# lightkurve/lightkurve

Hardware: AMD Instinct MI355X
Metric: frequencies*targets/sec (Lomb-Scargle, ls_method='fast' (reference default): extirpolation + FFT) + BLS periods*targets/sec; max-power rel-err (higher is better)
Workload: dtype f64

## Files before the change

### lightkurve_amd/csrc/ls_epilogue.hpp

```cpp
#pragma once
#include <hip/hip_runtime.h>

#include "../../include/lkhip.h"

namespace lk {

__device__ __forceinline__ double gls_power_sums(double Sh, double Ch, double S, double C, double S2, double C2,
                                                 int fit_mean, int norm, double YY, double psd_factor, double nN,
                                                 double scale) {
    double tan2;
    if (fit_mean)
        tan2 = (S2 - 2.0 * S * C) / (C2 - (C * C - S * S));
    else
        tan2 = S2 / C2;
    const double C2w = 1.0 / sqrt(1.0 + tan2 * tan2);
    const double S2w = tan2 * C2w;
    const double Cw = sqrt(0.5) * sqrt(1.0 + C2w);
    const double sgn = (S2w > 0.0) ? 1.0 : ((S2w < 0.0) ? -1.0 : 0.0);
    const double Sw = sqrt(0.5) * sgn * sqrt(1.0 - C2w);
    const double YC = Ch * Cw + Sh * Sw;
    const double YS = Sh * Cw - Ch * Sw;
    double CC = 0.5 * (1.0 + C2 * C2w + S2 * S2w);
    double SS = 0.5 * (1.0 - C2 * C2w - S2 * S2w);
    if (fit_mean) {
        const double a = C * Cw + S * Sw, bq = S * Cw - C * Sw;
        CC -= a * a;
        SS -= bq * bq;
    }
    double p = YC * YC / CC + YS * YS / SS;
    switch (norm) {
        case LK_NORM_STANDARD: p /= YY; break;
        case LK_NORM_PSD: p *= psd_factor; break;
        case LK_NORM_LK_AMPLITUDE: p = sqrt(p * psd_factor) * sqrt(4.0 / nN); break;
        default: p = p * psd_factor * scale; break;
    }
    return p;
}

__host__ __device__ __forceinline__ double rsqrt_refined(double x) {
#if defined(__HIP_DEVICE_COMPILE__)
    const double y = __builtin_amdgcn_rsq(x);
    const double e = fma(-(x * y), y, 1.0);
    return fma(y * e, fma(0.375, e, 0.5), y);
#else
    return 1.0 / sqrt(x);
#endif
}

__device__ __forceinline__ double gls_power_sums_lean(double Sh, double Ch, double S, double C, double S2, double C2,
                                                      int fit_mean, int norm, double YY, double psd_factor, double nN,
                                                      double scale) {
    double num = S2, den = C2;
    if (fit_mean) {
        num = S2 - 2.0 * S * C;
        den = C2 - (C * C - S * S);
    }
    double C2w, S2w;
    if (fmax(fabs(num), fabs(den)) >= 1e-150) {
        const double r = rsqrt_refined(num * num + den * den);
        C2w = fabs(den) * r;
        S2w = (den == 0.0) ? NAN : ((den < 0.0) ? -num : num) * r;
    } else {
        const double tan2 = num / den;
        C2w = 1.0 / sqrt(1.0 + tan2 * tan2);
        S2w = tan2 * C2w;
    }
    const double u = 0.5 + 0.5 * C2w;
    const double rc = rsqrt_refined(u);
    const double Cw = u * rc;
    const double Sw = 0.5 * S2w * rc;
    const double YC = Ch * Cw + Sh * Sw;
    const double YS = Sh * Cw - Ch * Sw;
    double CC = 0.5 * (1.0 + C2 * C2w + S2 * S2w);
    double SS = 0.5 * (1.0 - C2 * C2w - S2 * S2w);
    if (fit_mean) {
        const double a = C * Cw + S * Sw, bq = S * Cw - C * Sw;
        CC -= a * a;
        SS -= bq * bq;
    }
    double p = YC * YC / CC + YS * YS / SS;
    switch (norm) {
        case LK_NORM_STANDARD: p /= YY; break;
        case LK_NORM_PSD: p *= psd_factor; break;
        case LK_NORM_LK_AMPLITUDE: p = sqrt(p * psd_factor) * sqrt(4.0 / nN); break;
        default: p = p * psd_factor * scale; break;
    }
    return p;
}

template <int NT>
struct Chi2Sums {
    double Sw[2 * NT], Cw[2 * NT], Sy[NT], Cy[NT];
    __device__ __forceinline__ void zero() {
#pragma unroll
        for (int m = 0; m < 2 * NT; ++m) Sw[m] = Cw[m] = 0.0;
#pragma unroll
        for (int m = 0; m < NT; ++m) Sy[m] = Cy[m] = 0.0;
    }
    __device__ __forceinline__ void add(double a, double b, double w, double wy) {
        const double two_a = a + a;
        double cm = 1.0, sm = 0.0, c = a, s2 = b;
#pragma unroll
        for (int m = 0; m < 2 * NT; ++m) {
            Sw[m] = fma(w, s2, Sw[m]);
            Cw[m] = fma(w, c, Cw[m]);
            if (m < NT) {
                Sy[m] = fma(wy, s2, Sy[m]);
                Cy[m] = fma(wy, c, Cy[m]);
            }
            const double cn = fma(two_a, c, -cm), sn = fma(two_a, s2, -sm);
            cm = c;
            sm = s2;
            c = cn;
            s2 = sn;
        }
    }
    __device__ __forceinline__ void build(double yws, int fit_mean, double (&A)[2 * NT + 1][2 * NT + 1],
                                          double (&bv)[2 * NT + 1]) const {
        constexpr int D = 2 * NT + 1;
        auto CW = [&](int m) { return m == 0 ? 1.0 : Cw[m - 1]; };
        auto SW = [&](int m) { return m == 0 ? 0.0 : Sw[m - 1]; };
#pragma unroll
        for (int r = 0; r < D; ++r) {
            const int mr = (r + 1) >> 1;
            const bool rs = (r & 1) != 0;
            bv[r] = r == 0 ? yws : (rs ? Sy[mr - 1] : Cy[mr - 1]);
#pragma unroll
            for (int c = 0; c <= r; ++c) {
                const int mc = (c + 1) >> 1;
                const bool cs = (c & 1) != 0;
                const int dm = mr - mc, sm = mr + mc;
                double v;
                if (rs && cs)
                    v = 0.5 * (CW(dm) - CW(sm));
                else if (!rs && !cs)
                    v = 0.5 * (CW(dm) + CW(sm));
                else if (rs && !cs)
                    v = 0.5 * ((dm > 0 ? SW(dm) : 0.0) + SW(sm));
                else
                    v = 0.5 * ((dm > 0 ? -SW(dm) : 0.0) + SW(sm));
                A[r][c] = v;
            }
        }
        if (!fit_mean) {
            A[0][0] = 1.0;
            bv[0] = 0.0;
#pragma unroll
            for (int r = 1; r < D; ++r) A[r][0] = 0.0;
        }
    }
    __device__ __forceinline__ double solve_lu(double yws, int fit_mean) const {
        constexpr int D = 2 * NT + 1;
        double A[D][D], bv[D], b0[D];
        build(yws, fit_mean, A, bv);
#pragma unroll
        for (int r = 0; r < D; ++r) {
            b0[r] = bv[r];
#pragma unroll
            for (int c = r + 1; c < D; ++c) A[r][c] = A[c][r];
        }
        int perm[D];
#pragma unroll
        for (int r = 0; r < D; ++r) perm[r] = r;
#pragma unroll
        for (int j = 0; j < D; ++j) {
            int piv = j;
            double best = fabs(A[j][j]);
#pragma unroll
            for (int r = j + 1; r < D; ++r) {
                const double v = fabs(A[r][j]);
                if (v > best) {
                    best = v;
                    piv = r;
                }
            }
#pragma unroll
            for (int r = j + 1; r < D; ++r) {
                const bool sw = piv == r;
#pragma unroll
                for (int c = 0; c < D; ++c) {
                    const double x = A[j][c], y2 = A[r][c];
                    A[j][c] = sw ? y2 : x;
                    A[r][c] = sw ? x : y2;
                }
                const double x = bv[j], y2 = bv[r];
                bv[j] = sw ? y2 : x;
                bv[r] = sw ? x : y2;
            }
            const double inv = 1.0 / A[j][j];
#pragma unroll
            for (int r = j + 1; r < D; ++r) {
                const double f = A[r][j] * inv;
#pragma unroll
                for (int c = j + 1; c < D; ++c) A[r][c] = fma(-f, A[j][c], A[r][c]);
                bv[r] = fma(-f, bv[j], bv[r]);
            }
        }
        (void)perm;
        double x[D];
#pragma unroll
        for (int r = D - 1; r >= 0; --r) {
            double v = bv[r];
#pragma unroll
            for (int c = r + 1; c < D; ++c) v = fma(-A[r][c], x[c], v);
            x[r] = v / A[r][r];
        }
        double p = 0.0;
#pragma unroll
        for (int r = 0; r < D; ++r) p = fma(b0[r], x[r], p);
        return p;
    }
    __device__ __forceinline__ double solve(double yws, int fit_mean) const {
        constexpr int D = 2 * NT + 1;
        double A[D][D], bv[D];
        build(yws, fit_mean, A, bv);
        double p = 0.0;
#pragma unroll
        for (int j = 0; j < D; ++j) {
            double d = A[j][j];
#pragma unroll
            for (int m = 0; m < j; ++m) d = fma(-A[j][m], A[j][m], d);
            const double inv = 1.0 / sqrt(d);
            double z = bv[j];
#pragma unroll
            for (int m = 0; m < j; ++m) z = fma(-A[j][m], bv[m], z);
            z *= inv;
            bv[j] = z;
            p = fma(z, z, p);
#pragma unroll
            for (int r = j + 1; r < D; ++r) {
                double v = A[r][j];
#pragma unroll
                for (int m = 0; m < j; ++m) v = fma(-A[r][m], A[j][m], v);
                A[r][j] = v * inv;
            }
        }
        return p;
// ... 15 lines not shown
```

### lightkurve_amd/csrc/lsfast.hip

```cpp
#include <cmath>
#include <cstdlib>
#include <type_traits>
#include <vector>

#include "lk_common.hpp"
#include "ls_epilogue.hpp"

namespace lk {

typedef double lk_d2v __attribute__((ext_vector_type(2)));

constexpr int SPREAD_W = 1024;
constexpr int SPREAD_WW = 256;

struct FastStats {
    double wsum, ybar, YY, t0;
    double yws;
    double wmax;
    double vmax;
};

__device__ __forceinline__ void cadence_weights(const double *__restrict__ y, const double *__restrict__ dy, int64_t i,
                                                double wsum, double ybar, double &w, double &wy) {
    const double d = dy ? dy[i] : 1.0;
    w = (1.0 / (d * d)) / wsum;
    wy = w * (y[i] - ybar);
}

constexpr int PREP_NT = 512;
__global__ __launch_bounds__(PREP_NT) void lsf_prep_kernel(const double *__restrict__ t, const double *__restrict__ y,
                                                        const double *__restrict__ dy,
                                                        const int64_t *__restrict__ n_off, int center, int want_yy,
                                                        FastStats *__restrict__ stats, double df, int nfft, int m2,
                                                        int *__restrict__ rows_used) {
    constexpr int NT = PREP_NT;
    __shared__ double sh[NT / 64];
    const int b = blockIdx.x, tid = threadIdx.x;
    const int64_t lo = n_off[b], n = n_off[b + 1] - lo;
    auto breduce = [&](double x, auto op) {
#pragma unroll
        for (int o = 32; o > 0; o >>= 1) x = op(x, __shfl_xor(x, o));
        if ((tid & 63) == 0) sh[tid >> 6] = x;
        __syncthreads();
        double r = sh[0];
#pragma unroll
        for (int w = 1; w < NT / 64; ++w) r = op(r, sh[w]);
        __syncthreads();
        return r;
    };
    auto bsum = [&](double x) { return breduce(x, [](double a, double b2) { return a + b2; }); };
    auto bmax = [&](double x) { return breduce(x, [](double a, double b2) { return fmax(a, b2); }); };
    const double y0 = y[lo];
    double A = 0.0, Bz = 0.0, Cz = 0.0, tmin = INFINITY, tmax = -INFINITY;
    int unsorted = 0;
#pragma unroll 4
    for (int64_t i = tid; i < n; i += NT) {
        const double ti = t[lo + i], z = y[lo + i] - y0;
        double u = 1.0;
        if (dy) {
            const double d = dy[lo + i];
            u = 1.0 / (d * d);
        }
        A += u;
        Bz = fma(u, z, Bz);
        Cz = fma(u * z, z, Cz);
        tmin = fmin(tmin, ti);
        tmax = fmax(tmax, ti);
        if (i + 1 < n) unsorted |= (t[lo + i + 1] < ti) ? 1 : 0;
    }
    const double wsum = dy ? bsum(A) : (double)n;
    Bz = bsum(Bz);
    Cz = bsum(Cz);
    const double t0 = -bmax(-tmin);
    const double t1 = bmax(tmax);
    const int any_unsorted = __syncthreads_or(unsorted);
    const bool nowrap = (t1 - t0) * (double)nfft * df * 2.0 < (double)nfft - 8.0;
    const bool ordered = !any_unsorted && nowrap;
    if (rows_used) {
        if (tid < 3) {
            const double span = (t1 - t0) * (double)nfft * df * (tid == 2 ? 2.0 : 1.0);
            const int nrows = nfft >> m2;
            rows_used[b * 4 + tid] = (span >= (double)nfft - 8.0) ? nrows : min(nrows, (int)((span + 4.0) / (double)(1 << m2)) + 1);
        }
        if (tid == 0) rows_used[b * 4 + 3] = ordered ? 1 : 0;
    }
    const double delta = center ? Bz / wsum : 0.0;
    const double ybar = center ? y0 + delta : 0.0;
    double YY;
    if (want_yy) {
        double acc = 0.0;
        for (int64_t i = tid; i < n; i += NT) {
            const double d = dy ? dy[lo + i] : 1.0, r = y[lo + i] - ybar;
            acc = fma((1.0 / (d * d)) * r, r, acc);
        }
        YY = bsum(acc) / wsum;
    } else if (center) {
        YY = fmax(0.0, (Cz - Bz * delta) / wsum);
    } else {
        YY = (Cz + y0 * (2.0 * Bz + y0 * wsum)) / wsum;
    }
    double yws = 0.0, wmx = 0.0, vmx = 0.0;
    if (!(rows_used && ordered)) {
        double acc2 = 0.0;
        for (int64_t i = tid; i < n; i += NT) {
            double w, wy;
            cadence_weights(y, dy, lo + i, wsum, ybar, w, wy);
            acc2 += wy;
            wmx = fmax(wmx, w);
            vmx = fmax(vmx, fabs(wy));
        }
        yws = bsum(acc2);
        wmx = bmax(wmx);
        vmx = bmax(vmx);
    }
    if (tid == 0) stats[b] = FastStats{wsum, ybar, YY, t0, yws, wmx, vmx};
}

constexpr int TAB_PER_LANE = 8;
__global__ __launch_bounds__(256) void lsf_tables_kernel(const double *__restrict__ t, const int64_t *__restrict__ n_off,
                                                          const FastStats *__restrict__ stats,
                                                          const int *__restrict__ rows_used, double df, int nfft, int m2,
                                                          int logW, int *__restrict__ spread_tab, int ntab) {
    const int b = blockIdx.y;
    if (!rows_used[b * 4 + 3]) return;
    const int64_t lo = n_off[b], n = n_off[b + 1] - lo;
    const int lane = threadIdx.x & 63;
    const int64_t base = ((int64_t)blockIdx.x * 4 + (threadIdx.x >> 6)) * (64 * TAB_PER_LANE);
    if (base >= n) return;
    const double t0 = stats[b].t0;
    int *tab = spread_tab + (size_t)b * 4 * ntab;
    const double iW = 1.0 / (double)(1 << logW), dn = (double)nfft;
    auto posn = [&](double tt) {
        const double x = (tt - t0) * dn * df;
        return x < dn ? x : fmod(x, dn);
    };
    double p1[TAB_PER_LANE];
#pragma unroll
    for (int u = 0; u < TAB_PER_LANE; ++u) {
        const int64_t i = base + 64 * u + lane;
        p1[u] = posn(t[lo + (i < n ? i : n - 1)]);
    }
    const int nf0 = min(ntab, (int)((((long long)rows_used[b * 4 + 0] << m2) >> logW) + 3));
    const int nf2 = min(ntab, (int)((((long long)rows_used[b * 4 + 2] << m2) >> logW) + 3));
    double prev_last = base > 0 ? posn(t[lo + base - 1]) : -1e300;
#pragma unroll
    for (int u = 0; u < TAB_PER_LANE; ++u) {
        const int64_t i = base + 64 * u + lane;
        double pp1 = __shfl_up(p1[u], 1);
        if (lane == 0) pp1 = prev_last;
        prev_last = __shfl(p1[u], 63);
        if (i >= n) continue;
#pragma unroll
        for (int gg = 0; gg < 2; ++gg) {
            const double p = gg ? 2.0 * p1[u] : p1[u], pp = i > 0 ? (gg ? 2.0 * pp1 : pp1) : -1e300;
            int *lo_a = tab + (size_t)(2 * gg) * ntab, *hi_a = lo_a + ntab;
            const int nfill = gg ? nf2 : nf0;
            int k0 = i > 0 ? (int)floor((pp + 4.0) * iW) + 1 : 0, k1 = (int)floor((p + 4.0) * iW);
            for (int k = max(k0, 0); k <= min(k1, ntab - 1); ++k) lo_a[k] = (int)i;
            if (i == n - 1)
// ... 83 lines not shown
    const Quantum Qy = make_quantum(st.vmax), Qw = make_quantum(st.wmax);
    for (int fac = 1; fac <= 2; ++fac) {
        const double dff = df * (double)fac, f0f = f0 * (double)fac;
        double c = 1.0, s = 0.0;
        if (f0f > 0.0) phase_factor(f0f, tt, c, s);
        const Stencil4 sp = stencil4(fmod(tt * (double)nfft * dff, (double)nfft), nfft);
        if (fac == 1) {
            extirpolate4(g0, sp, wyi * c, wyi * s, Qy);
            if (fit_mean) extirpolate4(g1, sp, wi * c, wi * s, Qw);
        } else {
            extirpolate4(g2, sp, wi * c, wi * s, Qw);
        }
    }
}

__global__ __launch_bounds__(256) void lsf_spread_owner_kernel(const double *__restrict__ t, const double *__restrict__ y,
                                                                const double *__restrict__ dy,
                                                                const int64_t *__restrict__ n_off,
                                                                const FastStats *__restrict__ stats, int b0, double f0,
                                                                double df, int nfft, int m2, int fit_mean,
                                                                double2 *__restrict__ grids,
                                                                const int *__restrict__ rows_used,
                                                                const int *__restrict__ spread_tab, int ntab) {
    __shared__ double2 acc0[SPREAD_W], acc1[SPREAD_W];
    const int lb = blockIdx.y, tid = threadIdx.x;
    const bool pair = blockIdx.z == 0;
    if (!rows_used[lb * 4 + 3]) return;
    const int g = pair ? 0 : 2;
    const int ncell = rows_used[lb * 4 + g] << m2;
    const int c_lo = blockIdx.x * SPREAD_W, c_hi = min(c_lo + SPREAD_W, ncell);
    if (c_lo >= ncell) return;
    double2 *G0 = grids + ((size_t)lb * 3 + g) * (size_t)nfft, *G1 = G0 + nfft;
    const int b = b0 + lb;
    const int64_t lo = n_off[b];
    const FastStats st = stats[b];
    const double fac = pair ? 1.0 : 2.0;
    const double dff = df * fac, f0f = f0 * fac;
    for (int c = tid; c < SPREAD_W; c += 256) {
        acc0[c] = make_double2(0.0, 0.0);
        acc1[c] = make_double2(0.0, 0.0);
    }
    __syncthreads();
    const int lane = tid & 63, wv = tid >> 6;
    const int w_lo = c_lo + wv * SPREAD_WW, w_hi = min(w_lo + SPREAD_WW, c_hi);
    if (w_lo < w_hi) {
        const int *tab = spread_tab + ((size_t)b * 4 + (pair ? 0 : 2)) * ntab;
        const int kblk = blockIdx.x * (SPREAD_W / SPREAD_WW) + wv;
        const int i_lo = tab[kblk], i_hi = tab[ntab + min(kblk + 1, ntab - 1)];
        for (int i = i_lo + lane; i < i_hi; i += 64) {
            const double tt = t[lo + i] - st.t0;
            double wi, wyi;
            cadence_weights(y, dy, lo + i, st.wsum, st.ybar, wi, wyi);
            double c = 1.0, s = 0.0;
            if (f0f > 0.0) phase_factor(f0f, tt, c, s);
            const Stencil4 sp = stencil4(fmod(tt * (double)nfft * dff, (double)nfft), nfft);
            const double ar = (pair ? wyi : wi) * c, ai = (pair ? wyi : wi) * s, br = wi * c, bi = wi * s;
#pragma unroll
            for (int k = 0; k < 4; ++k) {
                const int cell = sp.i0 + k;
                if (k < sp.n && cell >= w_lo && cell < w_hi) {
                    unsafeAtomicAdd(&acc0[cell - c_lo].x, ar * sp.wt[k]);
                    unsafeAtomicAdd(&acc0[cell - c_lo].y, ai * sp.wt[k]);
                    if (pair && fit_mean) {
                        unsafeAtomicAdd(&acc1[cell - c_lo].x, br * sp.wt[k]);
                        unsafeAtomicAdd(&acc1[cell - c_lo].y, bi * sp.wt[k]);
                    }
                }
            }
        }
    }
    __syncthreads();
    for (int c = c_lo + tid; c < c_hi; c += 256) {
        G0[c] = acc0[c - c_lo];
        if (pair) G1[c] = acc1[c - c_lo];
    }
}

__device__ __forceinline__ void lds_fft_dit(double2 *x, const double2 *tw, int n, int m, int nf) {
    const int tid = threadIdx.x, nt = blockDim.x;
    const int halfn = n >> 1;
    for (int s = 1; s <= m; ++s) {
        const int half = 1 << (s - 1);
        const int tstep = n >> s;
        for (int p = tid; p < nf * halfn; p += nt) {
            const int f = p >> (m - 1), j = p & (halfn - 1);
            const int grp = j >> (s - 1), k = j & (half - 1);
            const int i0 = f * n + (grp << s) + k, i1 = i0 + half;
            const double2 wv = tw[k * tstep];
            const double2 a = x[i0], bq = x[i1];
            const double tr = wv.x * bq.x - wv.y * bq.y, ti = wv.x * bq.y + wv.y * bq.x;
            x[i0] = make_double2(a.x + tr, a.y + ti);
            x[i1] = make_double2(a.x - tr, a.y - ti);
        }
        __syncthreads();
    }
}

__device__ __forceinline__ void lds_twiddles(double2 *tw, int n) {
    for (int k = threadIdx.x; k < (n >> 1); k += blockDim.x) {
        double s, c;
        sincospi(2.0 * (double)k / (double)n, &s, &c);
        tw[k] = make_double2(c, s);
    }
}

__global__ __launch_bounds__(256) void fft_cols_kernel(double2 *__restrict__ grids, int m1, int m2, int CT) {
    extern __shared__ __attribute__((aligned(16))) double2 lds2[];
    const int N1 = 1 << m1, N2 = 1 << m2;
    double2 *x = lds2, *tw = lds2 + (size_t)CT * N1;
    double2 *G = grids + ((size_t)blockIdx.y << (m1 + m2));
    const int c0 = blockIdx.x * CT;
    lds_twiddles(tw, N1);
    for (int e = threadIdx.x; e < CT * N1; e += 256) {
        const int r = e / CT, cc = e - r * CT;
        const int rr = (int)(__brev((unsigned)r) >> (32 - m1));
        x[cc * N1 + rr] = G[(size_t)r * N2 + c0 + cc];
    }
    __syncthreads();
    lds_fft_dit(x, tw, N1, m1, CT);
    const double invN = 1.0 / (double)((size_t)1 << (m1 + m2));
    for (int e = threadIdx.x; e < CT * N1; e += 256) {
        const int k1 = e / CT, cc = e - k1 * CT;
        const long long ck = (long long)(c0 + cc) * k1;
        double s, c;
        sincospi(2.0 * (double)ck * invN, &s, &c);
        const double2 v = x[cc * N1 + k1];
        G[(size_t)k1 * N2 + c0 + cc] = make_double2(v.x * c - v.y * s, v.x * s + v.y * c);
    }
}

__global__ __launch_bounds__(256) void fft_rows_kernel(const double2 *__restrict__ grids, int m1, int m2, int RT,
                                                        int nkeep, double2 *__restrict__ spec) {
    extern __shared__ __attribute__((aligned(16))) double2 lds2[];
    const int N2 = 1 << m2;
    double2 *x = lds2, *tw = lds2 + (size_t)RT * N2;
    const double2 *G = grids + ((size_t)blockIdx.y << (m1 + m2));
    double2 *S = spec + (size_t)blockIdx.y * nkeep;
    const int r0 = blockIdx.x * RT;
    lds_twiddles(tw, N2);
    for (int e = threadIdx.x; e < RT * N2; e += 256) {
        const int rr = e / N2, c = e - rr * N2;
        const int cr = m2 ? (int)(__brev((unsigned)c) >> (32 - m2)) : 0;
        x[rr * N2 + cr] = G[(size_t)(r0 + rr) * N2 + c];
    }
    __syncthreads();
    lds_fft_dit(x, tw, N2, m2, RT);
    for (int e = threadIdx.x; e < RT * N2; e += 256) {
        const int k2 = e / RT, rr = e - k2 * RT;
        const long long k = (long long)(r0 + rr) + ((long long)k2 << m1);
        if (k < nkeep) S[k] = x[rr * N2 + k2];
    }
}

__device__ constexpr double R32C[16] = {1.0, 0.98078528040323043, 0.92387953251128674, 0.83146961230254524,
                                        0.70710678118654752, 0.55557023301960218, 0.38268343236508978,
                                        0.19509032201612825, 0.0, -0.19509032201612825, -0.38268343236508978,
                                        -0.55557023301960218, -0.70710678118654752, -0.83146961230254524,
                                        -0.92387953251128674, -0.98078528040323043};
__device__ constexpr double R32S[16] = {0.0, 0.19509032201612825, 0.38268343236508978, 0.55557023301960218,
                                        0.70710678118654752, 0.83146961230254524, 0.92387953251128674,
                                        0.98078528040323043, 1.0, 0.98078528040323043, 0.92387953251128674,
                                        0.83146961230254524, 0.70710678118654752, 0.55557023301960218,
                                        0.38268343236508978, 0.19509032201612825};

__host__ __device__ constexpr int brev_c(int x, int bits) {
    int r = 0;
    for (int i = 0; i < bits; ++i) r |= ((x >> i) & 1) << (bits - 1 - i);
    return r;
}

template <int L, bool UPPER_ZERO = false>
__device__ __forceinline__ void reg_fft(double2 (&v)[1 << L]) {
#pragma unroll
    for (int s = L; s >= 1; --s) {
        const int half = 1 << (s - 1);
#pragma unroll
        for (int g = 0; g < (1 << L); g += (1 << s)) {
#pragma unroll
            for (int k = 0; k < half; ++k) {
                const bool bz = UPPER_ZERO && s == L;
                const double2 a = v[g + k], b = bz ? make_double2(0.0, 0.0) : v[g + k + half];
                if (!bz) v[g + k] = make_double2(a.x + b.x, a.y + b.y);
                const double dx = bz ? a.x : a.x - b.x, dy = bz ? a.y : a.y - b.y;
                const int ti = k * (32 >> s);
                if (ti == 0)
                    v[g + k + half] = make_double2(dx, dy);
                else if (ti == 8)
                    v[g + k + half] = make_double2(-dy, dx);
                else
                    v[g + k + half] = make_double2(dx * R32C[ti] - dy * R32S[ti], dx * R32S[ti] + dy * R32C[ti]);
            }
        }
    }
}

__device__ __forceinline__ double2 cmul(double2 a, double2 b) {
    return make_double2(a.x * b.x - a.y * b.y, a.x * b.y + a.y * b.x);
}

template <int LA, int LB, int MODE, class Load, class Store>
__device__ __forceinline__ void block_fft(int NF, double2 *tile, Load load, Store store, int tw = 1) {
    constexpr int A = 1 << LA, Bq = 1 << LB, n = A * Bq, LDT = Bq + 1, FST = A * LDT + 1;
    const int tid = threadIdx.x;
    if (tid < NF * Bq) {
        int f, j;
        if (MODE == 1) {
            f = tid % NF;
            j = tid / NF;
        } else if (MODE == 2) {
            const int jl = tid % tw, rest = tid / tw;
            f = rest % NF;
            j = jl + tw * (rest / NF);
        } else {
            f = tid / Bq;
            j = tid % Bq;
        }
        double2 v[A];
#pragma unroll
        for (int i = 0; i < A; ++i) v[i] = load(f, i * Bq + j);
        reg_fft<LA>(v);
        double s1, c1;
        sincospi(2.0 * (double)j / (double)n, &s1, &c1);
        const double2 step = make_double2(c1, s1);
        double2 w = make_double2(1.0, 0.0);
        double2 *row = tile + (size_t)f * FST + j;
#pragma unroll
        for (int ka = 0; ka < A; ++ka) {
            row[ka * LDT] = cmul(v[brev_c(ka, LA)], w);
            w = cmul(w, step);
        }
    }
    __syncthreads();
    if (tid < NF * A) {
        const int ka = tid / NF, f = tid - ka * NF;
        const double2 *row = tile + (size_t)f * FST + (size_t)ka * LDT;
        double2 u[Bq];
#pragma unroll
        for (int j = 0; j < Bq; ++j) u[j] = row[j];
        reg_fft<LB>(u);
#pragma unroll
        for (int kb = 0; kb < Bq; ++kb) store(f, ka + A * kb, u[brev_c(kb, LB)], kb);
    }
}

template <int LA, int LB>
__global__ __launch_bounds__(256) void fft_cols_reg_kernel(double2 *__restrict__ grids, int m2, int CT,
                                                            const int *__restrict__ rows_used,
                                                            double2 *__restrict__ gout, int tw) {
    extern __shared__ __attribute__((aligned(16))) double2 lds2[];
    constexpr int m1 = LA + LB, A = 1 << LA;
    const int N2 = 1 << m2;
    double2 *G = grids + ((size_t)blockIdx.y << (m1 + m2));
    const int c0 = blockIdx.x * CT;
    const int ru = rows_used ? rows_used[(blockIdx.y / 3) * 4 + (blockIdx.y % 3)] : (1 << m1);
    const double invN = 1.0 / (double)((size_t)1 << (m1 + m2));
    auto load = [&](int f, int r) -> double2 {
        return r < ru ? G[(size_t)r * N2 + c0 + f] : make_double2(0.0, 0.0);
    };
    int last_f = -1;
    double2 w = make_double2(1.0, 0.0), step = w;
    const int twl = 31 - __clz(max(tw, 1));
    auto store = [&](int f, int k1, double2 v, int) {
        const int c = c0 + f;
        if (f != last_f) {
            double s, cc;
            sincospi(2.0 * (double)((long long)c * k1) * invN, &s, &cc);
            w = make_double2(cc, s);
            sincospi(2.0 * (double)((long long)c * A) * invN, &s, &cc);
            step = make_double2(cc, s);
            last_f = f;
        }
        if (gout)
            gout[((size_t)blockIdx.y << (m1 + m2)) + ((((size_t)(c >> twl) << m1) + k1) << twl) + (c & (tw - 1))] = cmul(v, w);
        else
            G[(size_t)k1 * N2 + c] = cmul(v, w);
        w = cmul(w, step);
    };
    block_fft<LA, LB, 1>(CT, lds2, load, store);
}

constexpr int PRUNED_CT = 16;
constexpr int LSF_LOG_NROOTS = 10, LSF_NROOTS = 1 << LSF_LOG_NROOTS;

constexpr int LSF_CHUNK_HALF_GB = 3;

template <int LP>
__global__ __launch_bounds__(PRUNED_CT * (1 << ((LP + 1) / 2)), 2) void fft_cols_pruned_kernel(
    const double2 *__restrict__ grids, int m1, int m2, const int *__restrict__ rows_used, double2 *__restrict__ gout,
    const double *__restrict__ t, const double *__restrict__ y, const double *__restrict__ dy,
    const int64_t *__restrict__ n_off, const FastStats *__restrict__ stats, int b0, double f0, double df, int fit_mean,
    const int *__restrict__ tab16, int ntab16, const double2 *__restrict__ roots) {
    extern __shared__ __attribute__((aligned(16))) double2 lds2[];
    constexpr int LA = (LP + 1) / 2, LB = LP / 2, A = 1 << LA, Bq = 1 << LB, P = 1 << LP, LDT = Bq + 1, FST = A * LDT + 1;
    constexpr int CT = PRUNED_CT, NT = CT * A;
    const int N1 = 1 << m1, N2 = 1 << m2, Q = N1 >> LP;
    const double2 *G = grids + ((size_t)blockIdx.y << (m1 + m2));
    const size_t tstride = (size_t)CT << m1, gstride = (size_t)(N2 / CT) * tstride;
    double2 *O = gout + (size_t)blockIdx.y * gstride + (size_t)blockIdx.x * tstride;
    const int c0 = blockIdx.x * CT;
    const int lbt = blockIdx.y / 3, g = blockIdx.y % 3;
    const int ru = rows_used[lbt * 4 + g];
    const int tid = threadIdx.x;
    const int f = tid % CT, jk = tid / CT;
    const bool p1 = jk < Bq, p2 = jk < A;
    const double invN = 1.0 / (double)((size_t)1 << (m1 + m2));
    const bool short_in = ru <= P / 2;
    double2 xin[A];
    if (tab16 != nullptr && rows_used[lbt * 4 + 3]) {
        double2 *acc = lds2;
        for (int e = tid; e < ru * CT; e += NT) acc[e] = make_double2(0.0, 0.0);
        __syncthreads();
        if (!(g == 1 && !fit_mean)) {
            const int b = b0 + lbt;
            const int64_t lo = n_off[b];
            const FastStats st = stats[b];
            const double fac = g == 2 ? 2.0 : 1.0, dff = df * fac, f0f = f0 * fac, dn = (double)((size_t)1 << (m1 + m2));
            const int nfft = 1 << (m1 + m2);
            const int *tlo = tab16 + ((size_t)b * 4 + (g == 2 ? 2 : 0)) * ntab16, *thi = tlo + ntab16;
            const int S = g == 2 ? 4 : 8, rpi = 64 / S;
            const int lane = tid & 63, wv = tid >> 6, rr = lane / S, k = lane - rr * S;
            const int rpw = (ru + NT / 64 - 1) / (NT / 64);
            const int r_end = min(ru, (wv + 1) * rpw);
            auto visit = [&](int r, double ti, double yi, double di) {
                const double tt = ti - st.t0;
                const double wi = (1.0 / (di * di)) / st.wsum, wyi = wi * (yi - st.ybar);
                double c = 1.0, sn = 0.0;
                if (f0f > 0.0) phase_factor(f0f, tt, c, sn);
                const double xp = tt * dn * dff;
                const Stencil4 sp = stencil4(xp < dn ? xp : fmod(xp, dn), nfft);
                const double amp = g == 0 ? wyi : wi, ar = amp * c, ai = amp * sn;
                const int cbase = (r << m2) + c0;
#pragma unroll
                for (int q = 0; q < 4; ++q) {
                    const unsigned col = (unsigned)(sp.i0 + q - cbase);
                    if (q < sp.n && col < (unsigned)CT) {
                        unsafeAtomicAdd(&acc[r * CT + col].x, ar * sp.wt[q]);
                        unsafeAtomicAdd(&acc[r * CT + col].y, ai * sp.wt[q]);
                    }
                }
            };
            constexpr int UN = 4;
            for (int rb = wv * rpw; rb < r_end; rb += UN * rpi) {
                int ii[UN], ih[UN];
#pragma unroll
                for (int u = 0; u < UN; ++u) {
                    const int r = rb + u * rpi + rr;
                    const int blk = (min(r, r_end - 1) << (m2 - 4)) + blockIdx.x;
// ... 226 lines not shown
    int lo = __double2loint(x), hi = __double2hiint(x);
    lo = __builtin_amdgcn_update_dpp(0, lo, 0x128, 0xF, 0xF, true);
    hi = __builtin_amdgcn_update_dpp(0, hi, 0x128, 0xF, 0xF, true);
    return __hiloint2double(hi, lo);
}

struct Rows512 {
    static constexpr int RT = 8;
    static constexpr int SK = 34;
    static constexpr int SF = 16 * SK + 4;
    static constexpr int NT = RT * 32;
    static constexpr size_t LDS_BYTES = (size_t)RT * SF * 8;
};

__global__ __launch_bounds__(Rows512::NT, 2) void fft_rows512_power_kernel(
    const double2 *__restrict__ grids, int m1, int ntargets, const int64_t *__restrict__ n_off,
    const FastStats *__restrict__ stats, int b0, double f0, double df, int64_t M, int fit_mean, int norm,
    const double *__restrict__ scale, double *__restrict__ power, PeakPart *__restrict__ peaks) {
    using R = Rows512;
    constexpr int RT = R::RT, SK = R::SK, SF = R::SF;
    extern __shared__ __attribute__((aligned(16))) double tile512[];
    const int tid = threadIdx.x;
    const size_t gstride = (size_t)1 << (m1 + 9);
    const int tiles_per_target = (1 << m1) / RT;
    const int jl = tid & 15, f1 = (tid >> 4) & (RT - 1), jh = tid >> 7, j = jl + 16 * jh;
    const int f2 = tid & 7, e = (tid >> 3) & 1, ka = tid >> 4;
    auto tile_base = [&](int T) {
        const int lbT = ntargets - 1 - T / tiles_per_target, r0T = (T % tiles_per_target) * RT;
        return grids + (size_t)lbT * 3 * gstride + ((size_t)jh << (m1 + 4)) + ((size_t)(r0T + f1) << 4) + jl;
    };
    double2 v[16];
    auto load = [&](const double2 *G) {
#pragma unroll
        for (int i = 0; i < 16; ++i) {
            const lk_d2v q = __builtin_nontemporal_load(reinterpret_cast<const lk_d2v *>(G + ((size_t)i << (m1 + 5))));
            v[i] = make_double2(q.x, q.y);
        }
    };
    double2 step1, step4;
    {
        double s, c;
        sincospi((double)j * (1.0 / 256.0), &s, &c);
        step1 = make_double2(c, s);
        sincospi((double)j * (1.0 / 64.0), &s, &c);
        step4 = make_double2(c, s);
    }
    double2 keep[3][4];
    const int k2need = (int)((M + ((int64_t)1 << m1) - 1) >> m1);
    const int nq = __builtin_amdgcn_readfirstlane(min(4, (k2need - 4 * (tid >> 6) + 31) >> 5));
    double *row1 = tile512 + f1 * SF + j;
    const double *row2 = tile512 + f2 * SF + ka * SK + e;
    auto process = [&](auto Gc, auto refill) {
        constexpr int G = decltype(Gc)::value;
        __builtin_amdgcn_sched_barrier(0);
        reg_fft<4>(v);
        __builtin_amdgcn_sched_barrier(0);
        {
            double2 w = step1;
#pragma unroll
            for (int bb = 1; bb < 4; ++bb) {
#pragma unroll
                for (int a = 0; a < 4; ++a) v[brev_c(4 * a + bb, 4)] = cmul(v[brev_c(4 * a + bb, 4)], w);
                if (bb < 3) w = cmul(w, step1);
            }
        }
        __builtin_amdgcn_sched_barrier(0);
        {
            double2 w = step4;
#pragma unroll
            for (int a = 1; a < 4; ++a) {
#pragma unroll
                for (int bb = 0; bb < 4; ++bb) v[brev_c(4 * a + bb, 4)] = cmul(v[brev_c(4 * a + bb, 4)], w);
                if (a < 3) w = cmul(w, step4);
            }
        }
        __builtin_amdgcn_sched_barrier(0);
        double ure[16], uim[16];
#pragma unroll
        for (int k = 0; k < 16; ++k) row1[k * SK] = v[brev_c(k, 4)].x;
        __syncthreads();
#pragma unroll
        for (int jj = 0; jj < 16; ++jj) ure[jj] = row2[2 * jj];
        __syncthreads();
#pragma unroll
        for (int k = 0; k < 16; ++k) row1[k * SK] = v[brev_c(k, 4)].y;
        __builtin_amdgcn_sched_barrier(0);
        refill();
        __syncthreads();
#pragma unroll
        for (int jj = 0; jj < 16; ++jj) uim[jj] = row2[2 * jj];
        __builtin_amdgcn_sched_barrier(0);
        double2 s0[8], s1[8];
#pragma unroll
        for (int q = 0; q < 8; ++q) {
            s0[q] = make_double2(ure[2 * q], uim[2 * q]);
            s1[q] = make_double2(ure[2 * q + 1], uim[2 * q + 1]);
        }
        reg_fft<3>(s0);
        __builtin_amdgcn_sched_barrier(0);
        reg_fft<3>(s1);
        __builtin_amdgcn_sched_barrier(0);
        auto pval = [&](int kb) -> double2 {
            const double2 a = s0[brev_c(kb, 3)], bq = s1[brev_c(kb, 3)];
            double2 hsum;
            if (kb == 0)
                hsum = make_double2(a.x + bq.x, a.y + bq.y);
            else if (kb == 4)
                hsum = make_double2(a.x - bq.y, a.y + bq.x);
            else
                hsum = make_double2(a.x + (bq.x * R32C[2 * kb] - bq.y * R32S[2 * kb]),
                                    a.y + (bq.x * R32S[2 * kb] + bq.y * R32C[2 * kb]));
            if (kb == 0) return hsum;
            const double wc = e ? R32C[kb] : 1.0, ws = e ? R32S[kb] : 0.0;
            return make_double2(hsum.x * wc - hsum.y * ws, hsum.x * ws + hsum.y * wc);
        };
#pragma unroll
        for (int q = 0; q < 4; ++q) {
            if (q < nq) {
                const double2 pev = pval(2 * q), pod = pval(2 * q + 1);
                const double2 mine = e ? pod : pev, send = e ? pev : pod;
                keep[G][q] = make_double2(mine.x + dpp_ror8(send.x), mine.y + dpp_ror8(send.y));
            }
            __builtin_amdgcn_sched_barrier(0);
        }
    };
    using I0 = std::integral_constant<int, 0>;
    using I1 = std::integral_constant<int, 1>;
    using I2 = std::integral_constant<int, 2>;
    const int T = blockIdx.x;
    const double2 *Gt = tile_base(T);
    load(Gt);
    {
        const int lb = ntargets - 1 - T / tiles_per_target, r0 = (T % tiles_per_target) * RT;
        process(I0{}, [&] { load(Gt + gstride); });
        __syncthreads();
        process(I1{}, [&] { load(Gt + 2 * gstride); });
        __syncthreads();
        process(I2{}, [] {});
        double best_v = 0.0;
        long long best_k = -1;
        {
            const int b = b0 + lb;
            const FastStats st = stats[b];
            const double nn = (double)(n_off[b + 1] - n_off[b]);
            const double sc = scale ? scale[b] : 1.0;
            const int k1 = r0 + f2;
            const double twopi = 6.283185307179586;
            double ph_c = 1.0, ph_s = 0.0, st_c = 1.0, st_s = 0.0;
            if (st.t0 != 0.0) {
                const long long kfirst = (long long)k1 + ((long long)(ka + 16 * e) << m1);
                sincos(twopi * st.t0 * (f0 + df * (double)kfirst), &ph_s, &ph_c);
                sincos(twopi * st.t0 * (df * (double)((long long)32 << m1)), &st_s, &st_c);
            }
#pragma unroll 1
            for (int q = 0; q < nq; ++q) {
                const long long k = (long long)k1 + ((long long)(ka + 16 * (2 * q + e)) << m1);
                if (k < M) {
                    double2 a = keep[0][0], bq = keep[1][0], c2 = keep[2][0];
                    if (st.t0 != 0.0) {
                        const double c = ph_c, s = ph_s;
                        a = make_double2(a.x * c - a.y * s, a.x * s + a.y * c);
                        bq = make_double2(bq.x * c - bq.y * s, bq.x * s + bq.y * c);
                        const double cc = c * c - s * s, ss = 2.0 * s * c;
                        c2 = make_double2(c2.x * cc - c2.y * ss, c2.x * ss + c2.y * cc);
                    }
                    const double pw = gls_power_sums_lean(a.y, a.x, bq.y, bq.x, c2.y, c2.x, fit_mean, norm, st.YY, 0.5 * st.wsum, nn, sc);
                    power[(size_t)b * (size_t)M + k] = pw;
                    if (pw == pw && peak_better(pw, k, best_v, best_k)) {
                        best_v = pw;
                        best_k = k;
                    }
                }
                const double nc = ph_c * st_c - ph_s * st_s, ns = ph_s * st_c + ph_c * st_s;
                ph_c = nc;
                ph_s = ns;
#pragma unroll
                for (int g = 0; g < 3; ++g)
#pragma unroll
                    for (int r = 0; r < 3; ++r) keep[g][r] = keep[g][r + 1];
            }
        }
        if (peaks != nullptr) {
#pragma unroll
            for (int o = 32; o > 0; o >>= 1) {
                const double v2 = __shfl_xor(best_v, o);
                const long long k2 = __shfl_xor(best_k, o);
                if (peak_better(v2, k2, best_v, best_k)) {
                    best_v = v2;
                    best_k = k2;
                }
            }
            if ((tid & 63) == 0)
                peaks[((size_t)lb * tiles_per_target + (T % tiles_per_target)) * (R::NT / 64) + (tid >> 6)] = PeakPart{best_v, best_k};
        }
    }
}

__global__ __launch_bounds__(64) void lsf_peaks_kernel(const PeakPart *__restrict__ peaks, int nparts, int b0,
                                                        double *__restrict__ max_out, int64_t *__restrict__ arg_out) {
    const PeakPart *pp = peaks + (size_t)blockIdx.x * nparts;
    double v = 0.0;
    long long k = -1;
    for (int i = threadIdx.x; i < nparts; i += 64)
        if (peak_better(pp[i].v, pp[i].k, v, k)) {
            v = pp[i].v;
            k = pp[i].k;
        }
#pragma unroll
    for (int o = 32; o > 0; o >>= 1) {
        const double v2 = __shfl_xor(v, o);
        const long long k2 = __shfl_xor(k, o);
        if (peak_better(v2, k2, v, k)) {
            v = v2;
            k = k2;
        }
    }
    if (threadIdx.x == 0) {
        max_out[b0 + blockIdx.x] = k >= 0 ? v : NAN;
        arg_out[b0 + blockIdx.x] = (int64_t)k;
    }
}

__global__ __launch_bounds__(256) void lsf_scatter_multi_kernel(const double *__restrict__ t, const double *__restrict__ y,
                                                                 const double *__restrict__ dy,
                                                                 const int64_t *__restrict__ n_off,
                                                                 const FastStats *__restrict__ stats, int b0, double f0,
                                                                 double df, int nfft, int nterms,
                                                                 double2 *__restrict__ grids) {
    const int b = b0 + blockIdx.y;
    const int64_t lo = n_off[b];
    const int n = (int)(n_off[b + 1] - lo);
    const int i = blockIdx.x * 256 + threadIdx.x;
    if (i >= n) return;
    const FastStats st = stats[b];
    const double tt = t[lo + i] - st.t0;
    double2 *g0 = grids + (size_t)blockIdx.y * 3 * nterms * nfft;
    double wi, wyi;
    cadence_weights(y, dy, lo + i, st.wsum, st.ybar, wi, wyi);
    const Quantum Qy = make_quantum(st.vmax), Qw = make_quantum(st.wmax);
    for (int fac = 1; fac <= 2 * nterms; ++fac) {
        const double dff = df * (double)fac, f0f = f0 * (double)fac;
        double c = 1.0, s = 0.0;
        if (f0f > 0.0) phase_factor(f0f, tt, c, s);
        const Stencil4 sp = stencil4(fmod(tt * (double)nfft * dff, (double)nfft), nfft);
        extirpolate4(g0 + (size_t)(nterms + fac - 1) * nfft, sp, wi * c, wi * s, Qw);
        if (fac <= nterms) extirpolate4(g0 + (size_t)(fac - 1) * nfft, sp, wyi * c, wyi * s, Qy);
    }
}

template <int NT>
__global__ __launch_bounds__(256) void lsf_chi2_power_kernel(const double2 *__restrict__ spec,
                                                              const int64_t *__restrict__ n_off,
                                                              const FastStats *__restrict__ stats, int b0, double f0,
                                                              double df, int64_t M, int fit_mean, int norm,
                                                              const double *__restrict__ scale,
                                                              double *__restrict__ power) {
    const int b = b0 + blockIdx.y;
    const int64_t j = (int64_t)blockIdx.x * 256 + threadIdx.x;
    if (j >= M) return;
    const FastStats st = stats[b];
    const double2 *s0 = spec + (size_t)blockIdx.y * 3 * NT * M;
    Chi2Sums<NT> sums;
    const double twopi = 6.283185307179586;
#pragma unroll
    for (int m = 1; m <= 2 * NT; ++m) {
        double cph = 1.0, sph = 0.0;
        if (st.t0 != 0.0) sincos(twopi * st.t0 * (double)m * (f0 + df * (double)j), &sph, &cph);
        const double2 a = s0[(size_t)(NT + m - 1) * M + j];
        sums.Cw[m - 1] = a.x * cph - a.y * sph;
        sums.Sw[m - 1] = a.x * sph + a.y * cph;
        if (m <= NT) {
            const double2 y = s0[(size_t)(m - 1) * M + j];
            sums.Cy[m - 1] = y.x * cph - y.y * sph;
            sums.Sy[m - 1] = y.x * sph + y.y * cph;
        }
    }
    const double n = (double)(n_off[b + 1] - n_off[b]);
    power[(size_t)b * (size_t)M + j] =
        chi2_normalise(sums.solve_lu(st.yws, fit_mean), norm, st.YY, 0.5 * st.wsum, n, scale ? scale[b] : 1.0);
}

__global__ __launch_bounds__(256) void lsf_power_kernel(const double2 *__restrict__ spec,
                                                         const int64_t *__restrict__ n_off,
                                                         const FastStats *__restrict__ stats, int b0, double f0,
                                                         double df, int64_t M, int fit_mean, int norm,
                                                         const double *__restrict__ scale,
                                                         double *__restrict__ power) {
    const int b = b0 + blockIdx.y;
    const int64_t j = (int64_t)blockIdx.x * 256 + threadIdx.x;
    if (j >= M) return;
    const FastStats st = stats[b];
    const double2 *s0 = spec + (size_t)blockIdx.y * 3 * M;
    double2 a = s0[j], bq = s0[M + j], c2 = s0[2 * M + j];
    if (st.t0 != 0.0) {
        const double twopi = 6.283185307179586;
        double s, c;
        sincos(twopi * st.t0 * (f0 + df * (double)j), &s, &c);
        a = make_double2(a.x * c - a.y * s, a.x * s + a.y * c);
        bq = make_double2(bq.x * c - bq.y * s, bq.x * s + bq.y * c);
        sincos(twopi * st.t0 * (2.0 * f0 + 2.0 * df * (double)j), &s, &c);
        c2 = make_double2(c2.x * c - c2.y * s, c2.x * s + c2.y * c);
    }
    const double n = (double)(n_off[b + 1] - n_off[b]);
    power[(size_t)b * (size_t)M + j] = gls_power_sums_lean(a.y, a.x, bq.y, bq.x, c2.y, c2.x, fit_mean, norm, st.YY,
                                                      0.5 * st.wsum, n, scale ? scale[b] : 1.0);
}

__global__ __launch_bounds__(256) void lsf_unquantize_kernel(double2 *__restrict__ grids, int m1, int m2,
                                                              const int *__restrict__ rows_used,
                                                              const FastStats *__restrict__ stats, int b0, int ngp, int n_wy) {
    const int lbt = blockIdx.y / ngp, g = blockIdx.y % ngp;
    if (rows_used && rows_used[lbt * 4 + 3]) return;
    const int ru = rows_used ? rows_used[lbt * 4 + g] : (1 << m1);
    const FastStats st = stats[b0 + lbt];
    const double q = make_quantum(g < n_wy ? st.vmax : st.wmax).q;
    if (!(q > 0.0)) return;
    const int N2 = 1 << m2;
    double2 *G = grids + ((size_t)blockIdx.y << (m1 + m2));
    for (int r = blockIdx.x * 8; r < min(blockIdx.x * 8 + 8, ru); ++r)
        for (int c = threadIdx.x; c < N2; c += 256) {
            const double2 v = G[(size_t)r * N2 + c];
            G[(size_t)r * N2 + c] = make_double2((double)__double_as_longlong(v.x) * q, (double)__double_as_longlong(v.y) * q);
        }
}

__global__ __launch_bounds__(256) void lsf_zero_kernel(double2 *__restrict__ grids, int m1, int m2,
                                                        const int *__restrict__ rows_used) {
    if (rows_used[(blockIdx.y / 3) * 4 + 3]) return;
    const int ru = rows_used[(blockIdx.y / 3) * 4 + (blockIdx.y % 3)];
    const int N2 = 1 << m2;
    double2 *G = grids + ((size_t)blockIdx.y << (m1 + m2));
    for (int r = blockIdx.x * 8; r < min(blockIdx.x * 8 + 8, ru); ++r)
// ... 475 lines not shown
```

Before: 10.17 billion.

## Use refined reciprocal/sqrt in LS power, tangent-form FFT butterflies, unroll epilogue loop

The Lomb-Scargle power epilogue replaces its two divisions with hardware reciprocal plus Newton refinement, and the amplitude sqrt with a refined rsqrt, when inputs are normal floats. The register FFT moves to a header and becomes decimation-in-time with bit-reversed indexing and tangent-based (cos*(b + tan*...)) FMA butterflies, which cuts multiplies per twiddle. The epilogue loop over q is fully unrolled to 4 and indexes keep[][q] directly instead of shifting the register array each iteration. These changes alter rounding slightly and rely on nq <= 4.

```diff
diff --git a/lightkurve_amd/csrc/ls_epilogue.hpp b/lightkurve_amd/csrc/ls_epilogue.hpp
--- a/lightkurve_amd/csrc/ls_epilogue.hpp
+++ b/lightkurve_amd/csrc/ls_epilogue.hpp
@@ -47,6 +47,30 @@
 #endif
 }
 
+__host__ __device__ __forceinline__ double rcp_refined(double x) {
+#if defined(__HIP_DEVICE_COMPILE__)
+    const double y = __builtin_amdgcn_rcp(x);
+    const double e = fma(-x, y, 1.0);
+    return fma(y, fma(e, e, e), y);
+#else
+    return 1.0 / x;
+#endif
+}
+
+__device__ __forceinline__ bool is_normal_f64(double x) { return __builtin_amdgcn_class(x, 0x008 | 0x100); }
+__device__ __forceinline__ bool is_positive_normal_f64(double x) { return __builtin_amdgcn_class(x, 0x100); }
+
+__device__ __forceinline__ double quotient_sum(double num1, double den1, double num2, double den2) {
+    const bool ok1 = is_normal_f64(den1), ok2 = is_normal_f64(den2);
+    if (ok1 && ok2) return fma(num1, rcp_refined(den1), num2 * rcp_refined(den2));
+    return num1 / den1 + num2 / den2;
+}
+
+__device__ __forceinline__ double sqrt_refined(double x) {
+    if (is_positive_normal_f64(x)) return x * rsqrt_refined(x);
+    return sqrt(x);
+}
+
 __device__ __forceinline__ double gls_power_sums_lean(double Sh, double Ch, double S, double C, double S2, double C2,
                                                       int fit_mean, int norm, double YY, double psd_factor, double nN,
                                                       double scale) {
@@ -78,11 +102,11 @@
         CC -= a * a;
         SS -= bq * bq;
     }
-    double p = YC * YC / CC + YS * YS / SS;
+    double p = quotient_sum(YC * YC, CC, YS * YS, SS);
     switch (norm) {
         case LK_NORM_STANDARD: p /= YY; break;
         case LK_NORM_PSD: p *= psd_factor; break;
-        case LK_NORM_LK_AMPLITUDE: p = sqrt(p * psd_factor) * sqrt(4.0 / nN); break;
+        case LK_NORM_LK_AMPLITUDE: p = sqrt_refined(p * psd_factor) * sqrt(4.0 / nN); break;
         default: p = p * psd_factor * scale; break;
     }
     return p;
diff --git a/lightkurve_amd/csrc/lsfast.hip b/lightkurve_amd/csrc/lsfast.hip
--- a/lightkurve_amd/csrc/lsfast.hip
+++ b/lightkurve_amd/csrc/lsfast.hip
@@ -5,6 +5,7 @@
 
 #include "lk_common.hpp"
 #include "ls_epilogue.hpp"
+#include "reg_fft.hpp"
 
 namespace lk {
 
@@ -394,47 +395,6 @@
     }
 }
 
-__device__ constexpr double R32C[16] = {1.0, 0.98078528040323043, 0.92387953251128674, 0.83146961230254524,
-                                        0.70710678118654752, 0.55557023301960218, 0.38268343236508978,
-                                        0.19509032201612825, 0.0, -0.19509032201612825, -0.38268343236508978,
-                                        -0.55557023301960218, -0.70710678118654752, -0.83146961230254524,
-                                        -0.92387953251128674, -0.98078528040323043};
-__device__ constexpr double R32S[16] = {0.0, 0.19509032201612825, 0.38268343236508978, 0.55557023301960218,
-                                        0.70710678118654752, 0.83146961230254524, 0.92387953251128674,
-                                        0.98078528040323043, 1.0, 0.98078528040323043, 0.92387953251128674,
-                                        0.83146961230254524, 0.70710678118654752, 0.55557023301960218,
-                                        0.38268343236508978, 0.19509032201612825};
-
-__host__ __device__ constexpr int brev_c(int x, int bits) {
-    int r = 0;
-    for (int i = 0; i < bits; ++i) r |= ((x >> i) & 1) << (bits - 1 - i);
-    return r;
-}
-
-template <int L, bool UPPER_ZERO = false>
-__device__ __forceinline__ void reg_fft(double2 (&v)[1 << L]) {
-#pragma unroll
-    for (int s = L; s >= 1; --s) {
-        const int half = 1 << (s - 1);
-#pragma unroll
-        for (int g = 0; g < (1 << L); g += (1 << s)) {
-#pragma unroll
-            for (int k = 0; k < half; ++k) {
-                const bool bz = UPPER_ZERO && s == L;
-                const double2 a = v[g + k], b = bz ? make_double2(0.0, 0.0) : v[g + k + half];
-                if (!bz) v[g + k] = make_double2(a.x + b.x, a.y + b.y);
-                const double dx = bz ? a.x : a.x - b.x, dy = bz ? a.y : a.y - b.y;
-                const int ti = k * (32 >> s);
-                if (ti == 0)
-                    v[g + k + half] = make_double2(dx, dy);
-                else if (ti == 8)
-                    v[g + k + half] = make_double2(-dy, dx);
-                else
-                    v[g + k + half] = make_double2(dx * R32C[ti] - dy * R32S[ti], dx * R32S[ti] + dy * R32C[ti]);
-            }
-        }
-    }
-}
 
 __device__ __forceinline__ double2 cmul(double2 a, double2 b) {
     return make_double2(a.x * b.x - a.y * b.y, a.x * b.y + a.y * b.x);
@@ -967,11 +927,12 @@
                 sincos(twopi * st.t0 * (f0 + df * (double)kfirst), &ph_s, &ph_c);
                 sincos(twopi * st.t0 * (df * (double)((long long)32 << m1)), &st_s, &st_c);
             }
-#pragma unroll 1
-            for (int q = 0; q < nq; ++q) {
+#pragma unroll
+            for (int q = 0; q < 4; ++q) {
+                if (q >= nq) break;
                 const long long k = (long long)k1 + ((long long)(ka + 16 * (2 * q + e)) << m1);
                 if (k < M) {
-                    double2 a = keep[0][0], bq = keep[1][0], c2 = keep[2][0];
+                    double2 a = keep[0][q], bq = keep[1][q], c2 = keep[2][q];
                     if (st.t0 != 0.0) {
                         const double c = ph_c, s = ph_s;
                         a = make_double2(a.x * c - a.y * s, a.x * s + a.y * c);
@@ -989,10 +950,6 @@
                 const double nc = ph_c * st_c - ph_s * st_s, ns = ph_s * st_c + ph_c * st_s;
                 ph_c = nc;
                 ph_s = ns;
-#pragma unroll
-                for (int g = 0; g < 3; ++g)
-#pragma unroll
-                    for (int r = 0; r < 3; ++r) keep[g][r] = keep[g][r + 1];
             }
         }
         if (peaks != nullptr) {
diff --git a/lightkurve_amd/csrc/reg_fft.hpp b/lightkurve_amd/csrc/reg_fft.hpp
--- /dev/null
+++ b/lightkurve_amd/csrc/reg_fft.hpp
@@ -0,0 +1,66 @@
+#pragma once
+#include <hip/hip_runtime.h>
+
+namespace lk {
+
+#if defined(__HIP_DEVICE_COMPILE__)
+#define LK_R32_TABLE __device__ constexpr
+#else
+#define LK_R32_TABLE static constexpr
+#endif
+LK_R32_TABLE double R32C[16] = {1.0, 0.98078528040323043, 0.92387953251128674, 0.83146961230254524,
+                                0.70710678118654752, 0.55557023301960218, 0.38268343236508978,
+                                0.19509032201612825, 0.0, -0.19509032201612825, -0.38268343236508978,
+                                -0.55557023301960218, -0.70710678118654752, -0.83146961230254524,
+                                -0.92387953251128674, -0.98078528040323043};
+LK_R32_TABLE double R32S[16] = {0.0, 0.19509032201612825, 0.38268343236508978, 0.55557023301960218,
+                                0.70710678118654752, 0.83146961230254524, 0.92387953251128674,
+                                0.98078528040323043, 1.0, 0.98078528040323043, 0.92387953251128674,
+                                0.83146961230254524, 0.70710678118654752, 0.55557023301960218,
+                                0.38268343236508978, 0.19509032201612825};
+LK_R32_TABLE double R32T[16] = {0.0, 0.19891236737965800691, 0.41421356237309504880, 0.66817863791929892000,
+                                1.0, 1.4966057626654890176, 2.4142135623730950488, 5.0273394921258481034,
+                                0.0, -5.0273394921258481034, -2.4142135623730950488, -1.4966057626654890176,
+                                -1.0, -0.66817863791929892000, -0.41421356237309504880, -0.19891236737965800691};
+#undef LK_R32_TABLE
+
+__host__ __device__ constexpr int brev_c(int x, int bits) {
+    int r = 0;
+    for (int i = 0; i < bits; ++i) r |= ((x >> i) & 1) << (bits - 1 - i);
+    return r;
+}
+
+template <int L, bool UPPER_ZERO = false>
+__host__ __device__ __forceinline__ void reg_fft(double2 (&v)[1 << L]) {
+#pragma unroll
+    for (int s = 1; s <= L; ++s) {
+        const int half = 1 << (s - 1);
+#pragma unroll
+        for (int g = 0; g < (1 << L); g += (1 << s)) {
+#pragma unroll
+            for (int k = 0; k < half; ++k) {
+                const int iu = brev_c(g + k, L), ib = brev_c(g + k + half, L);
+                if (UPPER_ZERO && s == 1) {
+                    v[ib] = v[iu];
+                    continue;
+                }
+                const double2 u = v[iu], b = v[ib];
+                const int ti = k * (32 >> s);
+                if (ti == 0) {
+                    v[iu] = make_double2(u.x + b.x, u.y + b.y);
+                    v[ib] = make_double2(u.x - b.x, u.y - b.y);
+                } else if (ti == 8) {
+                    v[iu] = make_double2(u.x - b.y, u.y + b.x);
+                    v[ib] = make_double2(u.x + b.y, u.y - b.x);
+                } else {
+                    const double c = R32C[ti], t = R32T[ti];
+                    const double s1 = fma(-t, b.y, b.x), s2 = fma(t, b.x, b.y);
+                    v[iu] = make_double2(fma(c, s1, u.x), fma(c, s2, u.y));
+                    v[ib] = make_double2(fma(-c, s1, u.x), fma(-c, s2, u.y));
+                }
+            }
+        }
+    }
+}
+
+}
```

Result: no change. 10.22 billion (median of 6 runs) (+0.5%).
